# p-m-mueller/saddle_point_petsc

Measured on AMD Instinct MI355X. Metric: FGMRES iterations/sec + achieved HBM GB/s on A-block SpMV, 1/2/4/8 MI355X, higher is better.
Workload: dtype f64

## Files before the change

saddle_point_petsc_amd/csrc/spk_device.hpp:

```cpp
#pragma once
#include "spk_internal.hpp"

#include <cmath>
#include <cstdlib>

namespace spk {
namespace k {

constexpr int kThreads = 256;
constexpr int kWave = 64;
constexpr int kVT = 1024;
constexpr int kVWaves = kVT / kWave;
constexpr int kVecUnroll = 4;
constexpr int kVecMaxBlocks = 256;

__device__ __forceinline__ double wave_sum(double v)
{
#pragma unroll
    for (int off = kWave / 2; off > 0; off >>= 1) v += __shfl_down(v, off, kWave);
    return v;
}

typedef double dbl2v __attribute__((ext_vector_type(2)));
typedef int int4v __attribute__((ext_vector_type(4)));
template <bool NT>
__device__ __forceinline__ double2 ld2s(const double *p, int64_t i2)
{
    if (NT) {
        const dbl2v v = __builtin_nontemporal_load(reinterpret_cast<const dbl2v *>(p) + i2);
        double2 r;
        r.x = v.x;
        r.y = v.y;
        return r;
    }
    return reinterpret_cast<const double2 *>(p)[i2];
}
__device__ __forceinline__ void st2nt(double *p, int64_t i2, double2 v)
// ... 437 lines not shown
        if (gr.ar.P) peer_allreduce_block(gr.ar, red, 1, gr.nrm2);
        else if (threadIdx.x == 0) gr.nrm2[0] = red[0];
        __syncthreads();
    }
    if (gr.sc && threadIdx.x == 0) gr.sc[gr.loc + 1] = inv_norm(*gr.nrm2);
    givens_block_lds<true>(gr.ka, gr.loc, gr.h, gr.nrm2, lds + kThreads, kMaxNv + 2, &pre);
}

void givens_rider_alone(const GivensRider &gr, const int32_t *done, hipStream_t s);
inline GivensRider no_rider()
{
    GivensRider g{};
    g.loc = -1;
    return g;
}

struct WsShape {
    int U, grid;
    bool on;
};
inline WsShape ws_shape(int64_t n2)
{
    WsShape v;
    static const int knob = [] { const char *e = getenv("SPK_VEC_WS"); return e ? atoi(e) : -1; }();
    v.on = n2 < (int64_t)kVecMaxBlocks * 2048 && knob != 0;
    v.U = n2 >= (int64_t)kVecMaxBlocks * 64 * 8 ? 8 : (n2 >= (int64_t)kVecMaxBlocks * 64 * 4 ? 4 : 2);
    if (knob == 2 || knob == 4 || knob == 8) v.U = knob;
    int64_t tiles = (n2 + 64 * v.U - 1) / (64 * v.U);
    if (tiles < 1) tiles = 1;
    v.grid = (int)(tiles < kVecMaxBlocks ? tiles : kVecMaxBlocks);
    return v;
}

template <int NG, int T, int G, bool NT, int U>
__device__ __forceinline__ void mdot_tiles(const double *__restrict__ V, int64_t ldv, int nv,
                                           const double *__restrict__ V2, int nv1,
                                           const double *__restrict__ w, int64_t n2,
                                           int64_t n_dot, double *__restrict__ partials,
                                           int with_ww, int split, double *lds)
{
    constexpr int NA = NG * 8 + 1, W = T / kWave, TILE2 = T * U;
    double acc[NA];
#pragma unroll
    for (int i = 0; i < NA; ++i) acc[i] = 0.0;

    for (int64_t tile = blockIdx.x; tile * TILE2 < n2; tile += gridDim.x) {
        double2 wv[U];
        int64_t idx[U];
#pragma unroll
        for (int u = 0; u < U; ++u) {
            idx[u] = tile * TILE2 + u * T + threadIdx.x;
            if (idx[u] < n2) {
                wv[u] = ld2(w, idx[u]);
                if (2 * idx[u] >= n_dot) wv[u].x = 0.0;
                if (2 * idx[u] + 1 >= n_dot) wv[u].y = 0.0;
            } else {
                wv[u].x = wv[u].y = 0.0;
                idx[u] = 0;
            }
        }
#pragma unroll
        for (int u = 0; u < U; ++u) acc[NA - 1] += wv[u].x * wv[u].x + wv[u].y * wv[u].y;
#pragma unroll
        for (int g0 = 0; g0 < NG * 8; g0 += G) {
            if (g0 < nv) {
                double2 a[G][U];
#pragma unroll
                for (int v = 0; v < G; ++v) {
                    const bool live = g0 + v < nv;
                    const int ic = live ? g0 + v : 0;
                    const int j2 = ic - nv1;
                    const double *Vi = !live ? w : (ic < nv1 ? V + (size_t)ic * ldv : V2 + (size_t)(split ? j2 >> 1 : j2) * ldv);
#pragma unroll
                    for (int u = 0; u < U; ++u) a[v][u] = ld2s<NT>(Vi, live ? idx[u] : 0);
                }
#pragma unroll
                for (int v = 0; v < G; ++v) {
                    const double mk = (g0 + v < nv) ? 1.0 : 0.0;
                    double d = 0.0;
                    if (split && g0 + v >= nv1 && g0 + v < nv) {
                        if ((g0 + v - nv1) & 1) {
#pragma unroll
                            for (int u = 0; u < U; ++u) d += a[v][u].y * wv[u].y;
                        } else {
#pragma unroll
                            for (int u = 0; u < U; ++u) d += a[v][u].x * wv[u].x;
                        }
                    } else {
#pragma unroll
                        for (int u = 0; u < U; ++u) d += a[v][u].x * wv[u].x + a[v][u].y * wv[u].y;
                    }
                    acc[g0 + v] += mk * d;
                }
            }
        }
    }
    const int lane = threadIdx.x & 63, wave = threadIdx.x >> 6;
#pragma unroll
    for (int i = 0; i < NA; ++i) {
        const double s = wave_sum(acc[i]);
        if (lane == 0) lds[wave * NA + i] = s;
    }
    __syncthreads();
    if (threadIdx.x < NA) {
        const int i = threadIdx.x;
        double s = 0.0;
#pragma unroll
        for (int j = 0; j < W; ++j) s += lds[j * NA + i];
        double *row = partials + (size_t)blockIdx.x * kPartialLd;
        if (i < nv) publish(row + i, s);
        else if (i == NA - 1 && with_ww) publish(row + nv, s);
    }
}

struct VecShape {
    int T, U, grid, G;
};
inline VecShape vec_shape(int64_t n2, bool maxpy = false)
{
    VecShape v;
    v.G = 4;
    int cap = kVecMaxBlocks;
    if (n2 >= (int64_t)kVecMaxBlocks * 2048) { v.T = 512; v.U = 4; }
    else if (n2 >= (int64_t)kVecMaxBlocks * 1024) { v.T = 256; v.U = 4; }
    else if (n2 >= (int64_t)kVecMaxBlocks * 512) { v.T = 256; v.U = 2; }
// ... 19 lines not shown
```

saddle_point_petsc_amd/csrc/spk_internal.hpp:

```cpp
#pragma once
#include <hip/hip_runtime.h>

#include <algorithm>
#include <chrono>
#include <cstdint>
#include <cstdio>
#include <functional>
#include <memory>
#include <string>
#include <vector>

#include <hip/hip_ext.h>

#include "../../include/spk.h"
#include "spk_amg.hpp"

namespace spk {

struct Error {
    int code;
    std::string msg;
};
[[noreturn]] void fail(int code, const char *fmt, ...);

// ... 436 lines not shown
};
struct IterB {
    const double *V;
    int64_t ldv;
    int nv;
    const double *dots;
    double *tb;
    double *w;
    const double *dinv, *bd;
    int64_t ldb;
    const double *shat, *gram;
    int fact;
    int64_t nl;
    int m, packed;
    double *zun;
    double *c;
    const double *wl_in;
    int lam_in_dot;
    double *partials, *out;
    PeerAR ar;
    int32_t *err;
    uint32_t fin_ticks;
    SendRanges sr;
    int gmain;
    const int32_t *done;
    double *sc, *hbuf, *wl_out;
    KrylovArrays ka;
    int loc;
    int defer_fin;
};
struct GsArgs {
    const double *V2;
    int cnt, split;
    int64_t n2, n_dot;
    double *partials;
    double *out;
    double *tot, *tot_next;
    FinErr fe;
};
int gs_fused(IterB b, GsArgs g, hipStream_t s);
int gs_fused_occupancy(int ng, int m);
int64_t gs_fused_grid(int64_t nl);
struct ResidentArgs {
    int mk, m, packed, fact, lam_in_dot;
    int64_t nl, ld;
    const double *V0, *V1;
    double *Z;
    const double *dinv, *bd;
    int64_t ldb;
    const double *shat, *gram;
    double *P;
    KrylovArrays ka;
    double *sc_out;
    int32_t *err;
    uint32_t ticks;
    PeerAR ar;
    SendRanges sr0, sr1;
    OffDiag od;
};
bool cycle_resident(const DictDev &A, int num_cus, ResidentArgs r, const int32_t *done, hipStream_t s);
int64_t resident_scratch_doubles(int num_cus, int mk);
bool resident_fits(const DictDev &A, int num_cus, int mk, int planes);
int iter_maxpy_uhead(IterB b, hipStream_t s);
template <class S>
struct Step {
    S *state;
    int mode;
    double *hist;
    int32_t hist_cap;
};
template <class S, class... Tau>
void state_init(S *state, const spk_opts &o, int norm, hipStream_t s, Tau... tau);
template <class S>
void state_scalar(Step<S> step, const double *sums, const int32_t *done, hipStream_t s);
// ... 104 lines not shown
    spk::DevBuf<double> bd;
    spk::DevBuf<double> bdpk;
    bool bd_packed = false;
    int inner_sweeps = 0;
    double inner_omega = 1.0;
    spk::DevBuf<float> a32, d32, x32, y32a, y32b;
    bool amg_on = false;
    spk_amg_opts amg_opts{};
    std::unique_ptr<spk_amg_hier> amg_h;
    std::unique_ptr<spk::AmgDev> amg_d;
    spk::DevBuf<double> bigdots;

    spk::DevBuf<double> partials;
    spk::DevBuf<double> small;
    spk::DevBuf<int32_t> errw;
    uint32_t fin_ticks = 400000000u;
    bool time_products = false;
    std::vector<hipEvent_t> tp_ev;
    size_t tp_used = 0;
    spk::k::Finish fin(double *out) { return spk::k::Finish{partials.p, out, spk::k::PeerAR{}, errw.p, fin_ticks}; }
    spk::k::Finish fin(double *out, const spk::k::PeerAR &ar) { return spk::k::Finish{partials.p, out, ar, errw.p, fin_ticks}; }
    void check_device_error();
    spk::DevBuf<double> y1tmp, ttmp;

    int last_form = -1, last_single = 0;

    int ws_restart = -1;
    spk::DevBuf<double> V, Z, xsol, rhs, tmp;
    spk::DevBuf<double> basis_sc;
    spk::DevBuf<double> res_P;
    int num_cus = 0;
    spk::DevBuf<double> gs_tot;
    uint32_t gs_seq = 0;
    int gs_occ[3] = {-1, -1, -1};
    bool gs_fused_fits(int64_t nl, int m);
    spk::SolverWork minres_work, pipecg_work;
    double pc_tau = SPK_PIPECGRR_TAU_DEFAULT;
    spk::DevBuf<double> kry_d;
    spk::DevBuf<spk::KrylovState> kst;
    spk::k::KrylovArrays ka{};

    spk::DevBuf<double> stage_x, stage_y;

    void ensure_scratch();
    void ensure_vectors();
    void upload_staged(void *dst, const void *src, size_t bytes);
    void *pin_state = nullptr;
    hipEvent_t state_ev = nullptr;
    void *pin[2] = {nullptr, nullptr};
    hipEvent_t pin_ev[2] = {nullptr, nullptr};
};

namespace spk {
void a_mult(spk_ctx *c, const double *x, double *y, const CsrDev *bt, const double *lam, const int32_t *done, bool accumulate,
            const k::OffDiag *od, const k::GivensRider *rider = nullptr);
void op_mult(spk_ctx *c, const double *x, double *y, const int32_t *done, bool halo_done = false, bool reuse_bt = false);
void op_pc_apply(spk_ctx *c, const double *x, double *y, const int32_t *done);
void pc_setup(spk_ctx *c, int pc_type, int schur_fact);
std::unique_ptr<spk_amg_hier> amg_build_ctx(spk_ctx *c);
void amg_upload(spk_ctx *c, std::unique_ptr<spk_amg_hier> h);
void amg_apply(spk_ctx *c, const double *x, double *y, int mode, const int32_t *done);
void fgmres(spk_ctx *c, const double *b_dev, double *x_dev, const spk_opts &o, spk_result *res,
            double *history, int32_t history_cap);
void minres(spk_ctx *c, const double *b_dev, double *x_dev, const spk_opts &o, int norm, spk_result *res,
            double *history, int32_t history_cap);
void pipecg(spk_ctx *c, const double *b_dev, double *x_dev, const spk_opts &o, int norm, spk_result *res,
            double *history, int32_t history_cap);
void pipecgrr(spk_ctx *c, const double *b_dev, double *x_dev, const spk_opts &o, int norm, double tau, spk_result *res,
// ... 80 lines not shown
```

saddle_point_petsc_amd/csrc/spk_k_iter.hip:

```cpp
#include "spk_device.hpp"

namespace spk {
namespace k {

template <int T, int G, int U, int MP, class Dots>
__device__ __forceinline__ void maxpy_uhead_tiles(const IterB &b, int scalar_wg, Dots dots)
{
    const int32_t dn = __builtin_nontemporal_load(b.done);
    __shared__ double hs[kMaxNv], lam[kMaxNv * 8], ys[8], wraws[8], tus[8];
    __shared__ double red[T];
    const int nv = b.nv, m = b.m;
    constexpr int NP = MP > 0 ? MP : 1;
    const int gmain = b.gmain;
    const bool is_main = (int)blockIdx.x < gmain;
    const int64_t n2 = b.nl / 2;
    const int bid = blockIdx.x;
    const int bx = b.sr.peer ? ((bid & 1) ? gmain - 1 - (bid >> 1) : (bid >> 1)) : bid;

    constexpr bool PRE = U * (MP > 0 ? MP : 1) <= 16;
    double2 wv[U], dv[U], pe[PRE ? NP : 1][U], t0[G][U];
    int64_t idx[U];
    bool ok[U];
    int64_t tile = bx;
    auto load_planes = [&]() {
#pragma unroll
        for (int q = 0; q < NP; ++q) {
            const bool live = b.packed ? 2 * q < m : q < m;
#pragma unroll
            for (int u = 0; u < U; ++u) {
                pe[q][u].x = pe[q][u].y = 0.0;
                if (live) pe[q][u] = ld2s<true>(b.bd + (size_t)q * b.ldb, idx[u]);
            }
        }
    };
    auto load_tile = [&](int64_t tl) {
#pragma unroll
        for (int u = 0; u < U; ++u) {
            idx[u] = tl * (T * U) + u * T + threadIdx.x;
            ok[u] = idx[u] < n2;
            if (!ok[u]) idx[u] = 0;
            wv[u] = ld2(b.w, idx[u]);
            dv[u] = ld2(b.dinv, idx[u]);
        }
        if (MP > 0 && PRE) load_planes();
#pragma unroll
        for (int v = 0; v < G; ++v) {
            const bool live = v < nv;
            const double *Vi = b.V + (size_t)(live ? v : 0) * b.ldv;
#pragma unroll
            for (int u = 0; u < U; ++u) t0[v][u] = ld2s<true>(Vi, live ? idx[u] : 0);
        }
    };
    bool have = is_main && tile * (T * U) < n2;
    if (have) load_tile(tile);

    double lamv = 0.0;
    const bool lam_mine = (int)threadIdx.x < nv * m;
    if (lam_mine) lamv = b.V[(size_t)(threadIdx.x / m) * b.ldv + b.nl + (threadIdx.x % m)];
    double wl = 0.0, sh = 1.0;
    if ((int)threadIdx.x < m) {
        wl = b.wl_in[threadIdx.x];
        sh = b.shat[threadIdx.x];
    }
    double hi_pre = 0.0, qv_pre = 0.0, tbv_pre[8], sci = 1.0;
    const double s_w = b.sc[nv - 1];
    if (threadIdx.x < kWave) {
        const int i = threadIdx.x;
        hi_pre = i < nv ? dots(i) : 0.0;
        sci = i < nv ? b.sc[i] : 0.0;
#pragma unroll
        for (int r = 0; r < 8; ++r) tbv_pre[r] = (r < m && i < nv) ? b.tb[i * 8 + r] : 0.0;
        qv_pre = (i < m) ? dots(nv + i) : 0.0;
    }
    if (dn) return;
    if (threadIdx.x < kWave) {
        const int i = threadIdx.x;
        const double hi = sci * s_w * hi_pre;
        const double ci = hi * sci;
        double tbv[8];
#pragma unroll
        for (int r = 0; r < 8; ++r) tbv[r] = tbv_pre[r] * sci;
        const double qv = qv_pre * s_w;
        if (i < nv) hs[i] = ci;
        if ((int)blockIdx.x == scalar_wg && i < nv) b.hbuf[i] = hi;
#pragma unroll
        for (int r = 0; r < 8; ++r) {
            if (r < m) {
// ... 44 lines not shown
        __syncthreads();
        double lam2 = 0.0;
        if (threadIdx.x == 0)
            for (int r = 0; r < m; ++r) lam2 += b.lam_in_dot ? wraws[r] * wraws[r] : 0.0;
        if (b.defer_fin) {
            if (threadIdx.x == 0) publish(b.partials + (size_t)gmain * kPartialLd, lam2);
            if (!is_main) return;
        } else {
            final_reduce(b.partials, gmain, kPartialLd, 1, red, FinErr{b.err, b.fin_ticks});
            if (threadIdx.x == 0) red[0] = red[0] + lam2;
            __syncthreads();
            if (b.ar.P) peer_allreduce_block(b.ar, red, 1, b.out);
            else if (threadIdx.x == 0) b.out[0] = red[0];
            return;
        }
    }
    if (!is_main) {
        const int64_t g = (int64_t)((int)blockIdx.x - gmain) * T + threadIdx.x;
        if (g < 2 * (int64_t)b.sr.nrecv) {
            uint32_t lo;
            const unsigned long long tw0 = (b.sr.stats && threadIdx.x == 0) ? wall_clock64() : 0ull;
            const bool okw = granule_wait(b.sr.mine + g, b.sr.seq, b.sr.timeout_ms, lo, b.sr.err, b.done);
            if (b.sr.stats && threadIdx.x == 0) {
                atomicAdd(b.sr.stats + 2 * kStatHalo, wall_clock64() - tw0);
                atomicAdd(b.sr.stats + 2 * kStatHalo + 1, 1ull);
            }
            const uint32_t other = __shfl_xor(lo, 1, kWave);
            if (!(g & 1)) b.sr.xghost[g >> 1] = join_halves(lo, other);
            if (!okw) raise_comm_error(b.sr.err, 18, b.sr.seq);
        }
        return;
    }
    double nrm = 0.0;
    while (have) {
        double2 sv[U];
#pragma unroll
        for (int u = 0; u < U; ++u) sv[u].x = sv[u].y = 0.0;
        if (MP > 0 && !PRE) {
#pragma unroll
            for (int q = 0; q < NP; ++q) {
                const bool live = b.packed ? 2 * q < m : q < m;
                if (live) {
#pragma unroll
                    for (int u = 0; u < U; ++u) {
                        const double2 e = ld2s<true>(b.bd + (size_t)q * b.ldb, idx[u]);
                        if (b.packed) {
                            sv[u].x += e.x * yv[2 * q];
                            sv[u].y += e.y * yv[2 * q + 1];
                        } else {
                            sv[u].x += e.x * yv[q];
                            sv[u].y += e.y * yv[q];
                        }
                    }
                }
            }
        } else if (MP > 0) {
            if (b.packed) {
#pragma unroll
                for (int q = 0; q < NP / 2; ++q) {
#pragma unroll
                    for (int u = 0; u < U; ++u) {
                        sv[u].x += pe[q][u].x * yv[2 * q];
                        sv[u].y += pe[q][u].y * yv[2 * q + 1];
                    }
                }
            } else {
#pragma unroll
                for (int r = 0; r < NP; ++r) {
#pragma unroll
                    for (int u = 0; u < U; ++u) {
                        sv[u].x += pe[r][u].x * yv[r];
                        sv[u].y += pe[r][u].y * yv[r];
                    }
                }
            }
        }
#pragma unroll
        for (int v = 0; v < G; ++v) {
            const double ai = v < nv ? -hs[v] : 0.0;
#pragma unroll
            for (int u = 0; u < U; ++u) {
                wv[u].x += ai * t0[v][u].x;
                wv[u].y += ai * t0[v][u].y;
            }
        }
        for (int g0 = G; g0 < nv; g0 += G) {
            double2 t[G][U];
            double ai[G];
#pragma unroll
            for (int v = 0; v < G; ++v) {
                const bool live = g0 + v < nv;
                const int ic = live ? g0 + v : 0;
                ai[v] = live ? -hs[ic] : 0.0;
                const double *Vi = b.V + (size_t)ic * b.ldv;
#pragma unroll
                for (int u = 0; u < U; ++u) t[v][u] = ld2s<true>(Vi, live ? idx[u] : 0);
            }
#pragma unroll
            for (int v = 0; v < G; ++v) {
#pragma unroll
                for (int u = 0; u < U; ++u) {
                    wv[u].x += ai[v] * t[v][u].x;
                    wv[u].y += ai[v] * t[v][u].y;
                }
            }
        }
#pragma unroll
        for (int u = 0; u < U; ++u) {
            if (ok[u]) {
                const int64_t i = idx[u];
                double2 zz, cc;
                nrm += wv[u].x * wv[u].x;
                nrm += wv[u].y * wv[u].y;
                zz.x = wv[u].x * dv[u].x;
                zz.y = wv[u].y * dv[u].y;
                if (MP > 0 && b.fact == SPK_SCHUR_FULL) {
                    zz.x -= sv[u].x;
                    zz.y -= sv[u].y;
                }
                st2nt(b.w, i, wv[u]);
                st2nt(b.zun, i, zz);
                if (MP > 0) {
                    cc.x = sv[u].x / dv[u].x;
                    cc.y = sv[u].y / dv[u].y;
                    st2nt(b.c, i, cc);
                }
                for (int q = 0; q < b.sr.n; ++q) {
                    const int64_t e = 2 * i - b.sr.r0[q];
                    if (b.sr.peer) {
                        const unsigned long long tag = (unsigned long long)b.sr.seq << 32;
                        if (e >= 0 && e < b.sr.len[q]) {
                            const unsigned long long bits = (unsigned long long)__double_as_longlong(zz.x);
                            st_sys(b.sr.remote[q] + 2 * e, tag | (bits & 0xffffffffull));
                            st_sys(b.sr.remote[q] + 2 * e + 1, tag | (bits >> 32));
                        }
                        if (e + 1 >= 0 && e + 1 < b.sr.len[q]) {
                            const unsigned long long bits = (unsigned long long)__double_as_longlong(zz.y);
                            st_sys(b.sr.remote[q] + 2 * e + 2, tag | (bits & 0xffffffffull));
                            st_sys(b.sr.remote[q] + 2 * e + 3, tag | (bits >> 32));
                        }
                    } else {
                        if (e >= 0 && e < b.sr.len[q]) b.sr.buf[b.sr.off[q] + e] = zz.x;
                        if (e + 1 >= 0 && e + 1 < b.sr.len[q]) b.sr.buf[b.sr.off[q] + e + 1] = zz.y;
                    }
                }
            }
        }
        tile += gmain;
        have = tile * (T * U) < n2;
        if (have) {
            load_tile(tile);
#pragma unroll
            for (int u = 0; u < U; ++u) {
                wv[u].x *= s_w;
                wv[u].y *= s_w;
            }
        }
    }
    const int lane = threadIdx.x & 63, wave = threadIdx.x >> 6;
    const double sw = wave_sum(nrm);
    if (lane == 0) red[wave] = sw;
    __syncthreads();
    if (threadIdx.x == 0) {
        double tsum = 0.0;
#pragma unroll
        for (int j = 0; j < T / kWave; ++j) tsum += red[j];
        publish(b.partials + (size_t)bx * kPartialLd, tsum);
    }
}
template <int T, int G, int U, int MP>
__global__ __launch_bounds__(T) void iter_maxpy_uhead_kernel(IterB b)
{
    const int nhalo = b.sr.peer ? (2 * b.sr.nrecv + T - 1) / T : 0;
    maxpy_uhead_tiles<T, G, U, MP>(b, b.gmain + nhalo, [&](int i) { return b.dots[i]; });
}

int iter_maxpy_uhead(IterB b, hipStream_t s)
{
    const int64_t n2 = b.nl / 2;
    const bool thin = n2 < (int64_t)kVecMaxBlocks * 2048;
    static const int t128 = [] { const char *e = getenv("SPK_B_T128"); return e ? atoi(e) : 0; }();
    const int U = thin ? (n2 < (int64_t)kVecMaxBlocks * 1024 ? 1 : 2) : 4;
    const bool tiny = thin && U == 1 && t128 && n2 <= (int64_t)1024 * 128;
    const int T = tiny ? 128 : (thin ? 256 : 512);
    int64_t tiles = (n2 + (int64_t)T * U - 1) / ((int64_t)T * U);
    if (tiles < 1) tiles = 1;
    b.gmain = (int)std::min<int64_t>(tiles, thin ? 1024 : kVecMaxBlocks);
    int grid = b.gmain + 1;
    if (b.sr.peer) grid += (2 * b.sr.nrecv + T - 1) / T;
    if (b.nv + b.m > kMaxNv - 1) fail(SPK_ERR_ARG, "iter_maxpy_uhead: %d values exceed one reduction", b.nv + b.m);
// ... 10 lines not shown
        else if (g1 == 16) SPK_IB(256, 16, 1, MPP);                              \
        else SPK_IB(256, 8, 1, MPP);                                             \
    } while (0)
    if (mp == 0) SPK_IB_MP(0);
    else if (mp == 4) SPK_IB_MP(4);
    else SPK_IB_MP(8);
#undef SPK_IB_MP
#undef SPK_IB
    return b.gmain;
}

struct TotalsWait {
    const double *tot;
    FinErr fe;
    __device__ double operator()(int i) const
    {
        double v = peek(tot + i);
        if (is_sentinel(v)) {
            const unsigned long long t0 = wall_clock64();
            do {
                __builtin_amdgcn_s_sleep(1);
                v = peek(tot + i);
            } while (is_sentinel(v) && wall_clock64() - t0 < (unsigned long long)fe.ticks &&
                     !(fe.err && __hip_atomic_load(fe.err, __ATOMIC_RELAXED, __HIP_MEMORY_SCOPE_AGENT)));
            if (is_sentinel(v) && fe.err) __hip_atomic_store(fe.err, 1, __ATOMIC_RELAXED, __HIP_MEMORY_SCOPE_AGENT);
        }
        return v;
    }
};

constexpr int kGsT = 512, kGsU = 4, kGsG = 4;

template <int NG, int MP>
__global__ __launch_bounds__(kGsT) void gs_fused_kernel(IterB b, GsArgs g)
{
    constexpr int NA = NG * 8 + 1, W = kGsT / kWave;
    __shared__ double lds[(W * NA > kGsT) ? W * NA : kGsT];
    if (blockIdx.x == 0 && threadIdx.x < kWave) publish(g.tot_next + threadIdx.x, __longlong_as_double((long long)kSentinelBits));
    if (*b.done) return;
    mdot_tiles<NG, kGsT, kGsG, true, kGsU>(b.V, b.ldv, g.cnt, g.V2, b.nv, b.w, g.n2, g.n_dot, g.partials, 1, g.split, lds);
    if (arrive_last(gridDim.x)) {
        const int k = g.cnt + 1;
        final_reduce(g.partials, gridDim.x, kPartialLd, k, lds, g.fe);
        if ((int)threadIdx.x < k) {
            g.out[threadIdx.x] = lds[threadIdx.x];
            publish(g.tot + threadIdx.x, lds[threadIdx.x]);
        }
    }
    maxpy_uhead_tiles<kGsT, kGsG, kGsU, MP>(b, (int)gridDim.x - 2, TotalsWait{g.tot, g.fe});
}

#define SPK_GS_SWITCH(NGV, MPV, CASE)                                                        \
    switch ((NGV) * 10 + (MPV)) {                                                           \
    case 10: CASE(1, 0); case 20: CASE(2, 0); case 30: CASE(3, 0); case 40: CASE(4, 0); case 50: CASE(5, 0); \
    case 14: CASE(1, 4); case 24: CASE(2, 4); case 34: CASE(3, 4); case 44: CASE(4, 4); case 54: CASE(5, 4); \
    case 18: CASE(1, 8); case 28: CASE(2, 8); case 38: CASE(3, 8); case 48: CASE(4, 8); default: CASE(5, 8); \
    }

int gs_fused_occupancy(int ng, int m)
{
    const int mp = m == 0 ? 0 : (m <= 4 ? 4 : 8);
    int nb = 0;
#define SPK_GS_OCC(NG, MP) SPK_HIP(hipOccupancyMaxActiveBlocksPerMultiprocessor(&nb, gs_fused_kernel<NG, MP>, kGsT, 0)); break
    SPK_GS_SWITCH(ng, mp, SPK_GS_OCC)
#undef SPK_GS_OCC
    return nb;
}

int64_t gs_fused_grid(int64_t nl)
{
    const int64_t n2 = nl / 2;
    if (n2 < (int64_t)kVecMaxBlocks * 2048) return 0;
    return kVecMaxBlocks;
}

int gs_fused(IterB b, GsArgs g, hipStream_t s)
{
    const int64_t grid = gs_fused_grid(b.nl);
    const VecShape vs = vec_shape(g.n2);
    if (!grid || vs.T != kGsT || vs.U != kGsU || vs.grid != grid) fail(SPK_ERR_STATE, "gs_fused: not the fat vector shape");
    if (!b.defer_fin || b.ar.P || b.sr.n || b.sr.peer) fail(SPK_ERR_STATE, "gs_fused: one rank, norm reduced by the rider only");
    if (g.cnt > 40 || b.nv + b.m > kMaxNv - 1) fail(SPK_ERR_ARG, "gs_fused: %d values exceed one reduction", g.cnt);
    b.gmain = (int)grid;
    const int ng = (g.cnt + 7) / 8 > 0 ? (g.cnt + 7) / 8 : 1;
    const int mp = b.m == 0 ? 0 : (b.m <= 4 ? 4 : 8);
#define SPK_GS_LAUNCH(NG, MP) hipLaunchKernelGGL((gs_fused_kernel<NG, MP>), dim3((unsigned)grid), dim3(kGsT), 0, s, b, g); break
    SPK_GS_SWITCH(ng, mp, SPK_GS_LAUNCH)
#undef SPK_GS_LAUNCH
    return b.gmain;
}
#undef SPK_GS_SWITCH

}
}
```

saddle_point_petsc_amd/csrc/spk_solver.cpp:

```cpp
#include <algorithm>
#include <chrono>
#include <cstddef>
#include <cstdlib>
#include <cstring>
#include <numeric>

#include "spk_internal.hpp"

using namespace spk;

void spk_ctx::ensure_scratch()
{
    if (!partials.p) {
        partials.alloc((size_t)k::kMaxBlocks * k::kPartialLd);
        k::arm_partials(partials.p, partials.n, stream);
        SPK_HIP(hipStreamSynchronize(stream));
    }
    if (!errw.p) errw.alloc(4);
    if (!small.p) small.alloc(512);
    if (!y1tmp.p) y1tmp.alloc(64);
    if (!ttmp.p) ttmp.alloc(64);
}

void spk_ctx::check_device_error()
{
    if (!errw.p) return;
    int32_t e = 0;
    SPK_HIP(hipMemcpy(&e, errw.p, sizeof e, hipMemcpyDeviceToHost));
    if (!e) return;
    SPK_HIP(hipStreamSynchronize(stream));
    SPK_HIP(hipMemset(errw.p, 0, sizeof(int32_t)));
    k::arm_partials(partials.p, partials.n, stream);
    if (gs_tot.p) k::arm_partials(gs_tot.p, gs_tot.n, stream);
    SPK_HIP(hipStreamSynchronize(stream));
    fail(SPK_ERR_HIP, "a cross-workgroup reduction timed out on the device (a workgroup never published its partial "
                      "sums within %.1f s): execution failure, the result of this call is not valid", fin_ticks / 1e8);
}

bool spk_ctx::gs_fused_fits(int64_t nl, int m)
{
    const int64_t grid = k::gs_fused_grid(nl);
    if (!grid) return false;
    const int mi = m == 0 ? 0 : (m <= 4 ? 1 : 2);
    if (gs_occ[mi] < 0) {
        int occ = 1 << 30;
        for (int ng = 1; ng <= 5; ++ng) occ = std::min(occ, k::gs_fused_occupancy(ng, m));
        gs_occ[mi] = occ;
    }
    return (int64_t)gs_occ[mi] * num_cus >= grid;
}

void spk_ctx::ensure_vectors()
{
    const int64_t want = ((int64_t)n_local + m + 255) / 256 * 256;
    if (want != ld) {
        ld = want;
        ws_restart = -1;
        tmp.release();
        tmpb.release();
        bt_cached = nullptr;
        stage_x.release();
        stage_y.release();
        xsol.release();
        rhs.release();
    }
    if (!tmp.p) tmp.alloc((size_t)ld);
    if (!xsol.p) xsol.alloc((size_t)ld);
    if (!rhs.p) rhs.alloc((size_t)ld);
    if (!stage_x.p) stage_x.alloc((size_t)ld);
    if (!stage_y.p) stage_y.alloc((size_t)ld);
}

void spk_ctx::upload_staged(void *dst, const void *src, size_t bytes)
{
    constexpr size_t kChunk = (size_t)32 << 20;
    if (bytes == 0) return;
    if (bytes < ((size_t)1 << 20)) {
        SPK_HIP(hipMemcpyAsync(dst, src, bytes, hipMemcpyHostToDevice, stream));
        SPK_HIP(hipStreamSynchronize(stream));
// ... 1083 lines not shown
    const int mk = o.restart;
    if (mk < 1 || mk > k::kBigNv - 2) fail(SPK_ERR_ARG, "fgmres: restart %d outside [1,%d]", mk, k::kBigNv - 2);
    const int32_t hist_cap = (int32_t)std::min<int64_t>((int64_t)std::max(o.max_it, 0) + 2, 1 << 22);
    if (c->ws_restart != mk) {
        c->V.alloc((size_t)c->ld * (mk + 2));
        c->Z.alloc((size_t)c->ld * (mk + 1));
        c->ws_restart = mk;
    }
    const int ldh = mk + 2;
    const size_t nd = (size_t)ldh * (mk + 1) + 4 * (size_t)(mk + 2) + 8 * (size_t)(mk + 2) + (size_t)hist_cap + 64;
    if (c->kry_d.n < nd) c->kry_d.alloc(nd);
    if (!c->kst.p) c->kst.alloc(1);
    double *p = c->kry_d.p;
    c->ka.st = c->kst.p;
    c->ka.ldh = ldh;
    c->ka.H = p;      p += (size_t)ldh * (mk + 1);
    c->ka.cc = p;     p += mk + 2;
    c->ka.ss = p;     p += mk + 2;
    c->ka.rs = p;     p += mk + 2;
    c->ka.nrs = p;    p += mk + 2;
    c->ka.hcol = nullptr;
    c->ka.tb = p;     p += 8 * (size_t)(mk + 2);
    c->ka.hist = p;
    c->ka.hist_cap = hist_cap;
}

namespace {
struct FgmresPlan {
    enum Product { kUn3, kSchurHead, kJacobiHead, kStep } product;
    enum Orth { kOrthUn3, kOrthMgs, kOrthSingle, kOrthCgs } orth;
    bool schur, head;
    bool big;
    bool resident, gsf;
    int chunk, refine;
    int nn, bpk, form;
    const double *bdp;
};

FgmresPlan plan_fgmres(spk_ctx *c, const spk_opts &o)
{
    FgmresPlan p{};
    const int mk = o.restart, m = c->m, nl = c->n_local;
    int form = o.iteration_form;
    if (const char *e = getenv("SPK_ITER_FORM")) {
        char *end = nullptr;
        const long f = strtol(e, &end, 10);
        if (end == e || *end || f < SPK_ITER_AUTO || f > SPK_ITER_LAST)
            fail(SPK_ERR_ARG, "SPK_ITER_FORM=%s: not an iteration form (%d..%d)", e, (int)SPK_ITER_AUTO, (int)SPK_ITER_LAST);
        form = (int)f;
    }
    if (form < SPK_ITER_AUTO || form > SPK_ITER_LAST) fail(SPK_ERR_ARG, "fgmres: unknown iteration_form %d", form);
    if (form == SPK_ITER_TWO_LAUNCH || form == SPK_ITER_THREE_LAUNCH || form == SPK_ITER_BA) form = SPK_ITER_UNNORM;
    p.big = mk > k::kMaxNv - 2;
    p.chunk = p.big ? 40 : k::kMaxNv;
    p.refine = o.cgs_refine;
    p.schur = o.fused && c->bd.p && c->pc_type == SPK_PC_SCHUR;
    const bool jac = o.fused && !p.schur && c->pc_type == SPK_PC_JACOBI && m == 0 && c->even_all && c->nonempty_all &&
                     c->inner_sweeps == 0 && !c->amg_d;
    p.head = p.schur || jac;
    p.nn = p.schur ? 1 + m : 1;
    p.bpk = p.schur && c->bd_packed ? 1 : 0;
    p.bdp = p.schur ? (p.bpk ? c->bdpk.p : c->bd.p) : nullptr;
    const bool cgs1 = o.orthog == SPK_ORTHOG_CGS && o.cgs_refine == SPK_REFINE_NEVER;
    const bool single = p.head && cgs1 && o.single_reduce == 1 && !p.big && mk + m <= k::kMaxNv - 1;
    const bool un3 = p.head && !single && cgs1 && mk + m <= k::kMaxNv - 2 &&
                     (form == SPK_ITER_UNNORM || form == SPK_ITER_AUTO || form == SPK_ITER_RESIDENT || form == SPK_ITER_GS_FUSED);
    static const bool res_env_off = [] { const char *e = getenv("SPK_RESIDENT"); return e && !strcmp(e, "0"); }();
    const int res_planes = !p.schur ? 0 : (p.bpk ? m / 2 : m);
    const bool res_multi = c->comm->size() > 1;
    const bool res_rank_ok = !res_multi ? (c->peers.empty() && c->n_ghost == 0)
                                        : (c->res_fit_all && c->comm->fuses() && (c->peers.empty() || c->send_ranges.n > 0));
    p.resident = un3 && (form == SPK_ITER_RESIDENT || (form == SPK_ITER_AUTO && !res_env_off)) && res_rank_ok &&
                 c->spmv_format == 1 && c->Adict.ok && c->Adict.bs == 2 && nl % 2 == 0 && mk >= (res_multi ? 3 : 2) &&
                 k::resident_fits(c->Adict, c->num_cus, mk, res_planes);
    p.gsf = un3 && !p.resident && (form == SPK_ITER_GS_FUSED || form == SPK_ITER_AUTO) && c->comm->size() == 1 &&
            c->peers.empty() && c->n_ghost == 0 && mk + m <= 41 && c->gs_fused_fits(nl, m);
    p.product = un3 ? FgmresPlan::kUn3 : p.schur ? FgmresPlan::kSchurHead : jac ? FgmresPlan::kJacobiHead : FgmresPlan::kStep;
    p.orth = un3 ? FgmresPlan::kOrthUn3 : o.orthog == SPK_ORTHOG_MGS ? FgmresPlan::kOrthMgs
           : single ? FgmresPlan::kOrthSingle : FgmresPlan::kOrthCgs;
    p.form = p.resident ? SPK_ITER_RESIDENT : p.gsf ? SPK_ITER_GS_FUSED : un3 ? SPK_ITER_UNNORM : p.head ? SPK_ITER_FOUR_LAUNCH : -1;
    return p;
}

void ensure_plan_buffers(spk_ctx *c, const FgmresPlan &p, int mk)
{
    if (p.big && c->bigdots.n < 2 * ((size_t)mk + 4)) c->bigdots.alloc(2 * ((size_t)mk + 4));
    const size_t need = p.resident ? (size_t)k::resident_scratch_doubles(c->num_cus, mk) : 0;
    if (c->res_P.n < need) c->res_P.alloc(need);
    if (p.gsf && !c->gs_tot.p) {
        c->gs_tot.alloc(2 * k::kPartialLd);
        k::arm_partials(c->gs_tot.p, c->gs_tot.n, c->stream);
    }
    if (p.product == FgmresPlan::kUn3 && c->basis_sc.n < (size_t)mk + 2) c->basis_sc.alloc((size_t)mk + 2);
}

struct FgmresRun {
    spk_ctx *c;
    const FgmresPlan &p;
    hipStream_t s;
    int mk, m, lam_in_dot, nl;
    int64_t N, ld, n_dot;
    double *V, *Z, *sm, *sm2, *nrm2b, *w1side;
    double *Vj(int j) const { return V + (size_t)ld * j; }
    double *Zj(int j) const { return Z + (size_t)ld * j; }
    double *dotsbuf(int q) const { return sm + (q & 1) * 128; }
    double *nrmbuf(int q) const { return sm + (q & 1) * 128 + 64; }
    double *wl(int q) const { return sm + 400 + (q & 1) * 8; }
};

// ... 52 lines not shown
            if (c->peers.empty()) a.sr0.n = a.sr1.n = 0;
            if (c->n_ghost > 0) a.od = c->offdiag();
        }
        if (!k::cycle_resident(c->Adict, c->num_cus, a, done, r.s)) fail(SPK_ERR_STATE, "fgmres: resident cycle kernel refused its shape");
        return true;
    }
    const bool gs = r.p.gsf && loc + 1 < r.mk;
    if (!gs) {
        const bool one = loc + 1 + r.m <= 40, spl = r.p.bpk && one;
        const k::PeerAR ar = one ? c->comm->fused_allreduce(loc + 2 + (schur ? r.m : 0), k::kStatArDots) : k::PeerAR{};
        k::mdot(r.V, r.ld, loc + 1, w, r.N, r.n_dot, c->fin(db, ar), done, r.s, schur ? (spl ? c->bdpk.p : c->bd.p) : nullptr,
                schur ? r.m : 0, spl ? 1 : 0);
        if (!ar.P) c->comm->allreduce_sum(db, loc + 2 + (schur ? r.m : 0), r.s);
    }
    const k::PeerAR ar2 = c->comm->fused_allreduce(1, k::kStatArNorm);
    k::IterB b{};
    b.V = r.V; b.ldv = r.ld; b.nv = loc + 1; b.dots = db; b.tb = c->ka.tb;
    b.w = w; b.dinv = c->dinv.p; b.bd = r.p.bdp; b.ldb = r.ld; b.shat = c->shat.p; b.gram = c->gram.p;
    b.fact = schur ? c->schur_fact : SPK_SCHUR_LOWER;
    b.nl = r.nl; b.m = r.m; b.packed = r.p.bpk;
    b.zun = r.Zj(loc + 1); b.c = schur ? r.Vj(loc + 2) : nullptr; b.wl_in = r.wl(loc); b.wl_out = r.wl(loc + 1);
    b.lam_in_dot = r.lam_in_dot;
    b.partials = c->partials.p; b.out = nb; b.ar = ar2; b.err = c->errw.p; b.fin_ticks = c->fin_ticks;
    b.sc = c->basis_sc.p; b.hbuf = r.sm2; b.ka = c->ka; b.loc = loc;
    const bool defer = loc + 1 < r.mk && (c->comm->size() == 1 || ar2.P);
    b.defer_fin = defer ? 1 : 0; b.done = done;
    k::SendRanges sr = c->send_ranges;
    const bool inb = sr.n > 0 && c->comm->fused_halo(sr, c->xghost.p);
    if (sr.n > 0) b.sr = sr;
    int fin_n;
    if (gs) {
        k::GsArgs g{};
        g.V2 = schur ? (r.p.bpk ? c->bdpk.p : c->bd.p) : nullptr;
        g.cnt = loc + 1 + (schur ? r.m : 0); g.split = r.p.bpk;
        g.n2 = (r.N + 1) / 2; g.n_dot = r.n_dot;
        g.partials = c->partials.p + 1;
        g.out = db;
        g.tot = c->gs_tot.p + (c->gs_seq & 1) * k::kPartialLd;
        g.tot_next = c->gs_tot.p + ((c->gs_seq + 1) & 1) * k::kPartialLd;
        g.fe = k::FinErr{c->errw.p, c->fin_ticks};
        fin_n = k::gs_fused(b, g, r.s);
        ++c->gs_seq;
    } else {
        fin_n = k::iter_maxpy_uhead(b, r.s);
    }
    if (!ar2.P && !defer) c->comm->allreduce_sum(nb, 1, r.s);
    k::GivensRider gr{c->ka, loc, r.sm2, nb, c->basis_sc.p, defer ? c->partials.p : nullptr, defer ? fin_n : 0,
                      k::FinErr{c->errw.p, c->fin_ticks}, defer ? ar2 : k::PeerAR{}};
    if (loc + 1 < r.mk) product(r, r.Zj(loc + 1), r.Vj(loc + 2), inb, schur, done, &gr);
    else cs.pend_h = r.sm2, cs.pend_n = nb, cs.pend_loc = loc;
    return false;
}

void head_product(const FgmresRun &r, CycleState &cs, int loc, double *w, const int32_t *done)
{
    spk_ctx *c = r.c;
    bool inhead = cs.prev_inhead;
    if (!cs.head_done) {
        k::SendRanges sr = c->send_ranges;
        inhead = sr.n > 0 && c->comm->fused_halo(sr, c->xghost.p);
        launch_head(r, loc, w, r.p.big ? -1 : loc - 1, sr.n > 0 && (r.p.schur || inhead) ? &sr : nullptr, done, nullptr);
        cs.last = r.p.big ? -1 : loc;
        if (r.p.schur && r.p.orth == FgmresPlan::kOrthSingle) k::copy_small(w + r.nl, r.wl(loc), r.m, done, r.s);
    }
    if (r.p.schur) product(r, r.Zj(loc), w, inhead, true, done);
    else op_mult(c, r.Zj(loc), w, done, inhead);
}
// ... 186 lines not shown
```

Before: 6481.

## Keep first-tile w, parity planes and leading basis vectors between dot and maxpy phases

In the fused Gram-Schmidt kernel, the first tile that each block handles in the mdot phase now keeps its w values, packed parity planes and first four basis vectors in registers or LDS. The maxpy phase then reads them from there instead of fetching them again from HBM. This saves one re-read per block of its first tile across the grid-wide reduction wait. The cost is extra registers and shared memory, which may lower occupancy and so shrink or disable the gs_fused path, whose fit check now depends on the keep variant.

Result: faster. 6595, median of 6 (+1.8%).

```diff
diff --git a/saddle_point_petsc_amd/csrc/spk_device.hpp b/saddle_point_petsc_amd/csrc/spk_device.hpp
--- a/saddle_point_petsc_amd/csrc/spk_device.hpp
+++ b/saddle_point_petsc_amd/csrc/spk_device.hpp
@@ -3,6 +3,7 @@
 
 #include <cmath>
 #include <cstdlib>
+#include <type_traits>
 
 namespace spk {
 namespace k {
@@ -506,19 +507,45 @@
     return v;
 }
 
-template <int NG, int T, int G, bool NT, int U>
+struct NoKeep {
+    static constexpr int KW = 0, KP = 0, KV = 0;
+    static constexpr bool any = false;
+    __device__ __forceinline__ void put(int, int, double2) {}
+    __device__ __forceinline__ double2 get(int, int) const { return double2{0.0, 0.0}; }
+};
+template <int T, int U, int KW_, int KP_, int KV_, int KR_>
+struct KeepSet {
+    static constexpr int KW = KW_, KP = KP_, KV = KV_, KR = KR_, N = KW_ + KP_ + KV_, KL = N > KR_ ? N - KR_ : 0;
+    static constexpr bool any = N > 0;
+    double2 r[KR_ > 0 ? KR_ : 1][U];
+    double2 *l;
+    __device__ __forceinline__ void put(int k, int u, double2 v)
+    {
+        if (k < KR) r[k][u] = v;
+        else l[((k - KR) * U + u) * T + threadIdx.x] = v;
+    }
+    __device__ __forceinline__ double2 get(int k, int u) const
+    {
+        return k < KR ? r[k][u] : l[((k - KR) * U + u) * T + threadIdx.x];
+    }
+};
+
+template <int NG, int T, int G, bool NT, int U, class Keep = NoKeep>
 __device__ __forceinline__ void mdot_tiles(const double *__restrict__ V, int64_t ldv, int nv,
                                            const double *__restrict__ V2, int nv1,
                                            const double *__restrict__ w, int64_t n2,
                                            int64_t n_dot, double *__restrict__ partials,
-                                           int with_ww, int split, double *lds)
+                                           int with_ww, int split, double *lds, Keep *keep = nullptr)
 {
     constexpr int NA = NG * 8 + 1, W = T / kWave, TILE2 = T * U;
+    constexpr int KW = Keep::KW, KP = Keep::KP, KV = Keep::KV;
     double acc[NA];
 #pragma unroll
     for (int i = 0; i < NA; ++i) acc[i] = 0.0;
 
     for (int64_t tile = blockIdx.x; tile * TILE2 < n2; tile += gridDim.x) {
+        const bool KF = Keep::any && tile == (int64_t)blockIdx.x;
+        const bool kpl = KF && KP > 0 && split && nv > nv1;
         double2 wv[U];
         int64_t idx[U];
 #pragma unroll
@@ -526,6 +553,7 @@
             idx[u] = tile * TILE2 + u * T + threadIdx.x;
             if (idx[u] < n2) {
                 wv[u] = ld2(w, idx[u]);
+                if (KF && KW) keep->put(0, u, wv[u]);
                 if (2 * idx[u] >= n_dot) wv[u].x = 0.0;
                 if (2 * idx[u] + 1 >= n_dot) wv[u].y = 0.0;
             } else {
@@ -533,6 +561,18 @@
                 idx[u] = 0;
             }
         }
+        if (kpl) {
+#pragma unroll
+            for (int q = 0; q < KP; ++q) {
+                const bool live = nv1 + 2 * q < nv;
+#pragma unroll
+                for (int u = 0; u < U; ++u) {
+                    double2 e{0.0, 0.0};
+                    if (live) e = ld2s<NT>(V2 + (size_t)q * ldv, idx[u]);
+                    keep->put(KW + q, u, e);
+                }
+            }
+        }
 #pragma unroll
         for (int u = 0; u < U; ++u) acc[NA - 1] += wv[u].x * wv[u].x + wv[u].y * wv[u].y;
 #pragma unroll
@@ -541,7 +581,7 @@
                 double2 a[G][U];
 #pragma unroll
                 for (int v = 0; v < G; ++v) {
-                    const bool live = g0 + v < nv;
+                    const bool live = g0 + v < nv && !(kpl && g0 + v >= nv1 && ((g0 + v - nv1) >> 1) < KP);
                     const int ic = live ? g0 + v : 0;
                     const int j2 = ic - nv1;
                     const double *Vi = !live ? w : (ic < nv1 ? V + (size_t)ic * ldv : V2 + (size_t)(split ? j2 >> 1 : j2) * ldv);
@@ -550,9 +590,10 @@
                 }
 #pragma unroll
                 for (int v = 0; v < G; ++v) {
-                    const double mk = (g0 + v < nv) ? 1.0 : 0.0;
+                    const bool live = g0 + v < nv && !(kpl && g0 + v >= nv1 && ((g0 + v - nv1) >> 1) < KP);
+                    const double mk = live ? 1.0 : 0.0;
                     double d = 0.0;
-                    if (split && g0 + v >= nv1 && g0 + v < nv) {
+                    if (split && g0 + v >= nv1 && live) {
                         if ((g0 + v - nv1) & 1) {
 #pragma unroll
                             for (int u = 0; u < U; ++u) d += a[v][u].y * wv[u].y;
@@ -565,6 +606,37 @@
                         for (int u = 0; u < U; ++u) d += a[v][u].x * wv[u].x + a[v][u].y * wv[u].y;
                     }
                     acc[g0 + v] += mk * d;
+                }
+                if (KF && g0 < KV) {
+#pragma unroll
+                    for (int v = 0; v < G; ++v) {
+                        if (g0 + v < KV && g0 + v < nv1) {
+#pragma unroll
+                            for (int u = 0; u < U; ++u) keep->put(KW + KP + g0 + v, u, a[v][u]);
+                        }
+                    }
+                }
+            }
+        }
+        if (kpl) {
+#pragma unroll
+            for (int q = 0; q < KP; ++q) {
+#pragma unroll
+                for (int h = 0; h < 2; ++h) {
+                    const int slot = nv1 + 2 * q + h;
+                    if (slot < nv) {
+                        double d = 0.0;
+                        if (h) {
+#pragma unroll
+                            for (int u = 0; u < U; ++u) d += keep->get(KW + q, u).y * wv[u].y;
+                        } else {
+#pragma unroll
+                            for (int u = 0; u < U; ++u) d += keep->get(KW + q, u).x * wv[u].x;
+                        }
+#pragma unroll
+                        for (int i = 0; i < NA - 1; ++i)
+                            if (i == slot) acc[i] += d;
+                    }
                 }
             }
         }
diff --git a/saddle_point_petsc_amd/csrc/spk_internal.hpp b/saddle_point_petsc_amd/csrc/spk_internal.hpp
--- a/saddle_point_petsc_amd/csrc/spk_internal.hpp
+++ b/saddle_point_petsc_amd/csrc/spk_internal.hpp
@@ -492,6 +492,7 @@
 struct GsArgs {
     const double *V2;
     int cnt, split;
+    int keep;
     int64_t n2, n_dot;
     double *partials;
     double *out;
@@ -499,7 +500,7 @@
     FinErr fe;
 };
 int gs_fused(IterB b, GsArgs g, hipStream_t s);
-int gs_fused_occupancy(int ng, int m);
+int gs_fused_occupancy(int ng, int m, bool keep);
 int64_t gs_fused_grid(int64_t nl);
 struct ResidentArgs {
     int mk, m, packed, fact, lam_in_dot;
@@ -670,8 +671,8 @@
     int num_cus = 0;
     spk::DevBuf<double> gs_tot;
     uint32_t gs_seq = 0;
-    int gs_occ[3] = {-1, -1, -1};
-    bool gs_fused_fits(int64_t nl, int m);
+    int gs_occ[6] = {-1, -1, -1, -1, -1, -1};
+    bool gs_fused_fits(int64_t nl, int m, bool keep);
     spk::SolverWork minres_work, pipecg_work;
     double pc_tau = SPK_PIPECGRR_TAU_DEFAULT;
     spk::DevBuf<double> kry_d;
diff --git a/saddle_point_petsc_amd/csrc/spk_k_iter.hip b/saddle_point_petsc_amd/csrc/spk_k_iter.hip
--- a/saddle_point_petsc_amd/csrc/spk_k_iter.hip
+++ b/saddle_point_petsc_amd/csrc/spk_k_iter.hip
@@ -3,9 +3,11 @@
 namespace spk {
 namespace k {
 
-template <int T, int G, int U, int MP, class Dots>
-__device__ __forceinline__ void maxpy_uhead_tiles(const IterB &b, int scalar_wg, Dots dots)
-{
+template <int T, int G, int U, int MP, class Dots, class Keep = NoKeep>
+__device__ __forceinline__ void maxpy_uhead_tiles(const IterB &b, int scalar_wg, Dots dots, Keep *keep = nullptr)
+{
+    constexpr int KW = Keep::KW, KP = Keep::KP, KV = Keep::KV;
+    static_assert(KV % G == 0, "whole groups of basis vectors are kept");
     const int32_t dn = __builtin_nontemporal_load(b.done);
     __shared__ double hs[kMaxNv], lam[kMaxNv * 8], ys[8], wraws[8], tus[8];
     __shared__ double red[T];
@@ -18,7 +20,9 @@
     const int bx = b.sr.peer ? ((bid & 1) ? gmain - 1 - (bid >> 1) : (bid >> 1)) : bid;
 
     constexpr bool PRE = U * (MP > 0 ? MP : 1) <= 16;
-    double2 wv[U], dv[U], pe[PRE ? NP : 1][U], t0[G][U];
+    static_assert(KP == 0 || (PRE && KP <= NP / 2), "kept planes are parity planes fetched ahead");
+    const bool kpl = KP > 0 && b.packed && m > 0;
+    double2 wv[U], dv[U], pe[PRE ? NP : 1][U], t0[G][U], tdead;
     int64_t idx[U];
     bool ok[U];
     int64_t tile = bx;
@@ -33,26 +37,38 @@
             }
         }
     };
-    auto load_tile = [&](int64_t tl) {
+    auto load_tile = [&](int64_t tl, bool KF) {
 #pragma unroll
         for (int u = 0; u < U; ++u) {
             idx[u] = tl * (T * U) + u * T + threadIdx.x;
             ok[u] = idx[u] < n2;
             if (!ok[u]) idx[u] = 0;
-            wv[u] = ld2(b.w, idx[u]);
+            wv[u] = KF && KW ? keep->get(0, u) : ld2(b.w, idx[u]);
             dv[u] = ld2(b.dinv, idx[u]);
         }
-        if (MP > 0 && PRE) load_planes();
+        if (MP > 0 && PRE) {
+            if (KF && kpl) {
+#pragma unroll
+                for (int q = 0; q < NP; ++q) {
+#pragma unroll
+                    for (int u = 0; u < U; ++u) pe[q][u] = q < KP ? keep->get(KW + q, u) : double2{0.0, 0.0};
+                }
+            } else {
+                load_planes();
+            }
+        }
+        if (KF && KV > 0) tdead = ld2s<true>(b.V, 0);
+        const int v0 = KF ? KV : 0;
 #pragma unroll
         for (int v = 0; v < G; ++v) {
-            const bool live = v < nv;
-            const double *Vi = b.V + (size_t)(live ? v : 0) * b.ldv;
+            const bool live = v0 + v < nv;
+            const double *Vi = b.V + (size_t)(live ? v0 + v : 0) * b.ldv;
 #pragma unroll
             for (int u = 0; u < U; ++u) t0[v][u] = ld2s<true>(Vi, live ? idx[u] : 0);
         }
     };
     bool have = is_main && tile * (T * U) < n2;
-    if (have) load_tile(tile);
+    if (have) load_tile(tile, Keep::any);
 
     double lamv = 0.0;
     const bool lam_mine = (int)threadIdx.x < nv * m;
@@ -163,7 +179,9 @@
         return;
     }
     double nrm = 0.0;
+    bool KF = Keep::any;
     while (have) {
+        const int v0 = KF ? KV : 0;
         double2 sv[U];
 #pragma unroll
         for (int u = 0; u < U; ++u) sv[u].x = sv[u].y = 0.0;
@@ -207,15 +225,31 @@
             }
         }
 #pragma unroll
-        for (int v = 0; v < G; ++v) {
-            const double ai = v < nv ? -hs[v] : 0.0;
-#pragma unroll
-            for (int u = 0; u < U; ++u) {
-                wv[u].x += ai * t0[v][u].x;
-                wv[u].y += ai * t0[v][u].y;
-            }
-        }
-        for (int g0 = G; g0 < nv; g0 += G) {
+        for (int s = 0; s < KV; ++s) {
+            if (KF && (s < G || s / G * G < nv)) {
+                const bool live = s < nv;
+                const double ai = live ? -hs[s] : 0.0;
+#pragma unroll
+                for (int u = 0; u < U; ++u) {
+                    double2 tk = tdead;
+                    if (live) tk = keep->get(KW + KP + s, u);
+                    wv[u].x += ai * tk.x;
+                    wv[u].y += ai * tk.y;
+                }
+            }
+        }
+        if (v0 == 0 || v0 < nv) {
+#pragma unroll
+            for (int v = 0; v < G; ++v) {
+                const double ai = v0 + v < nv ? -hs[v0 + v] : 0.0;
+#pragma unroll
+                for (int u = 0; u < U; ++u) {
+                    wv[u].x += ai * t0[v][u].x;
+                    wv[u].y += ai * t0[v][u].y;
+                }
+            }
+        }
+        for (int g0 = v0 + G; g0 < nv; g0 += G) {
             double2 t[G][U];
             double ai[G];
 #pragma unroll
@@ -280,13 +314,14 @@
         tile += gmain;
         have = tile * (T * U) < n2;
         if (have) {
-            load_tile(tile);
+            load_tile(tile, false);
 #pragma unroll
             for (int u = 0; u < U; ++u) {
                 wv[u].x *= s_w;
                 wv[u].y *= s_w;
             }
         }
+        KF = false;
     }
     const int lane = threadIdx.x & 63, wave = threadIdx.x >> 6;
     const double sw = wave_sum(nrm);
@@ -363,13 +398,23 @@
 constexpr int kGsT = 512, kGsU = 4, kGsG = 4;
 
 template <int NG, int MP>
+struct GsKeep {
+    static constexpr int KP = MP == 4 && NG <= 4 ? 2 : 0, KV = 4;
+    using type = KeepSet<kGsT, kGsU, 1, KP, KV, 1 + KP>;
+};
+
+template <int NG, int MP, bool KEEP>
 __global__ __launch_bounds__(kGsT) void gs_fused_kernel(IterB b, GsArgs g)
 {
     constexpr int NA = NG * 8 + 1, W = kGsT / kWave;
+    using Keep = typename std::conditional<KEEP, typename GsKeep<NG, MP>::type, KeepSet<kGsT, kGsU, 0, 0, 0, 0>>::type;
     __shared__ double lds[(W * NA > kGsT) ? W * NA : kGsT];
+    __shared__ double2 klds[Keep::KL > 0 ? Keep::KL * kGsU * kGsT : 1];
+    Keep keep;
+    keep.l = klds;
     if (blockIdx.x == 0 && threadIdx.x < kWave) publish(g.tot_next + threadIdx.x, __longlong_as_double((long long)kSentinelBits));
     if (*b.done) return;
-    mdot_tiles<NG, kGsT, kGsG, true, kGsU>(b.V, b.ldv, g.cnt, g.V2, b.nv, b.w, g.n2, g.n_dot, g.partials, 1, g.split, lds);
+    mdot_tiles<NG, kGsT, kGsG, true, kGsU>(b.V, b.ldv, g.cnt, g.V2, b.nv, b.w, g.n2, g.n_dot, g.partials, 1, g.split, lds, &keep);
     if (arrive_last(gridDim.x)) {
         const int k = g.cnt + 1;
         final_reduce(g.partials, gridDim.x, kPartialLd, k, lds, g.fe);
@@ -378,7 +423,7 @@
             publish(g.tot + threadIdx.x, lds[threadIdx.x]);
         }
     }
-    maxpy_uhead_tiles<kGsT, kGsG, kGsU, MP>(b, (int)gridDim.x - 2, TotalsWait{g.tot, g.fe});
+    maxpy_uhead_tiles<kGsT, kGsG, kGsU, MP>(b, (int)gridDim.x - 2, TotalsWait{g.tot, g.fe}, &keep);
 }
 
 #define SPK_GS_SWITCH(NGV, MPV, CASE)                                                        \
@@ -388,11 +433,14 @@
     case 18: CASE(1, 8); case 28: CASE(2, 8); case 38: CASE(3, 8); case 48: CASE(4, 8); default: CASE(5, 8); \
     }
 
-int gs_fused_occupancy(int ng, int m)
+int gs_fused_occupancy(int ng, int m, bool keep)
 {
     const int mp = m == 0 ? 0 : (m <= 4 ? 4 : 8);
     int nb = 0;
-#define SPK_GS_OCC(NG, MP) SPK_HIP(hipOccupancyMaxActiveBlocksPerMultiprocessor(&nb, gs_fused_kernel<NG, MP>, kGsT, 0)); break
+#define SPK_GS_OCC(NG, MP)                                                                                          \
+    if (keep) SPK_HIP(hipOccupancyMaxActiveBlocksPerMultiprocessor(&nb, gs_fused_kernel<NG, MP, true>, kGsT, 0));  \
+    else SPK_HIP(hipOccupancyMaxActiveBlocksPerMultiprocessor(&nb, gs_fused_kernel<NG, MP, false>, kGsT, 0));      \
+    break
     SPK_GS_SWITCH(ng, mp, SPK_GS_OCC)
 #undef SPK_GS_OCC
     return nb;
@@ -415,7 +463,10 @@
     b.gmain = (int)grid;
     const int ng = (g.cnt + 7) / 8 > 0 ? (g.cnt + 7) / 8 : 1;
     const int mp = b.m == 0 ? 0 : (b.m <= 4 ? 4 : 8);
-#define SPK_GS_LAUNCH(NG, MP) hipLaunchKernelGGL((gs_fused_kernel<NG, MP>), dim3((unsigned)grid), dim3(kGsT), 0, s, b, g); break
+#define SPK_GS_LAUNCH(NG, MP)                                                                                       \
+    if (g.keep) hipLaunchKernelGGL((gs_fused_kernel<NG, MP, true>), dim3((unsigned)grid), dim3(kGsT), 0, s, b, g);  \
+    else hipLaunchKernelGGL((gs_fused_kernel<NG, MP, false>), dim3((unsigned)grid), dim3(kGsT), 0, s, b, g);        \
+    break
     SPK_GS_SWITCH(ng, mp, SPK_GS_LAUNCH)
 #undef SPK_GS_LAUNCH
     return b.gmain;
diff --git a/saddle_point_petsc_amd/csrc/spk_solver.cpp b/saddle_point_petsc_amd/csrc/spk_solver.cpp
--- a/saddle_point_petsc_amd/csrc/spk_solver.cpp
+++ b/saddle_point_petsc_amd/csrc/spk_solver.cpp
@@ -37,14 +37,14 @@
                       "sums within %.1f s): execution failure, the result of this call is not valid", fin_ticks / 1e8);
 }
 
-bool spk_ctx::gs_fused_fits(int64_t nl, int m)
+bool spk_ctx::gs_fused_fits(int64_t nl, int m, bool keep)
 {
     const int64_t grid = k::gs_fused_grid(nl);
     if (!grid) return false;
-    const int mi = m == 0 ? 0 : (m <= 4 ? 1 : 2);
+    const int mi = (m == 0 ? 0 : (m <= 4 ? 1 : 2)) + (keep ? 3 : 0);
     if (gs_occ[mi] < 0) {
         int occ = 1 << 30;
-        for (int ng = 1; ng <= 5; ++ng) occ = std::min(occ, k::gs_fused_occupancy(ng, m));
+        for (int ng = 1; ng <= 5; ++ng) occ = std::min(occ, k::gs_fused_occupancy(ng, m, keep));
         gs_occ[mi] = occ;
     }
     return (int64_t)gs_occ[mi] * num_cus >= grid;
@@ -1194,6 +1194,7 @@
     bool schur, head;
     bool big;
     bool resident, gsf;
+    int gs_keep;
     int chunk, refine;
     int nn, bpk, form;
     const double *bdp;
@@ -1235,8 +1236,10 @@
     p.resident = un3 && (form == SPK_ITER_RESIDENT || (form == SPK_ITER_AUTO && !res_env_off)) && res_rank_ok &&
                  c->spmv_format == 1 && c->Adict.ok && c->Adict.bs == 2 && nl % 2 == 0 && mk >= (res_multi ? 3 : 2) &&
                  k::resident_fits(c->Adict, c->num_cus, mk, res_planes);
+    const char *keep_env = getenv("SPK_GS_KEEP");
+    p.gs_keep = keep_env && !strcmp(keep_env, "0") ? 0 : 1;
     p.gsf = un3 && !p.resident && (form == SPK_ITER_GS_FUSED || form == SPK_ITER_AUTO) && c->comm->size() == 1 &&
-            c->peers.empty() && c->n_ghost == 0 && mk + m <= 41 && c->gs_fused_fits(nl, m);
+            c->peers.empty() && c->n_ghost == 0 && mk + m <= 41 && c->gs_fused_fits(nl, m, p.gs_keep != 0);
     p.product = un3 ? FgmresPlan::kUn3 : p.schur ? FgmresPlan::kSchurHead : jac ? FgmresPlan::kJacobiHead : FgmresPlan::kStep;
     p.orth = un3 ? FgmresPlan::kOrthUn3 : o.orthog == SPK_ORTHOG_MGS ? FgmresPlan::kOrthMgs
            : single ? FgmresPlan::kOrthSingle : FgmresPlan::kOrthCgs;
@@ -1355,7 +1358,7 @@
     if (gs) {
         k::GsArgs g{};
         g.V2 = schur ? (r.p.bpk ? c->bdpk.p : c->bd.p) : nullptr;
-        g.cnt = loc + 1 + (schur ? r.m : 0); g.split = r.p.bpk;
+        g.cnt = loc + 1 + (schur ? r.m : 0); g.split = r.p.bpk; g.keep = r.p.gs_keep;
         g.n2 = (r.N + 1) / 2; g.n_dot = r.n_dot;
         g.partials = c->partials.p + 1;
         g.out = db;
```
